# OpenDriveLab/OccNet

Measured on AMD Instinct MI355X. Metric: nuScenes samples/sec (6-cam 900x1600 -> 200x200x16 voxels), higher is better.
Workload: dtype f32 hot path (GEMM operands bf16x3-split, SCA value rows q16 block floating point) + bf16 backbone; 1 GPU; bevformer_base_occ forward: 6x(3x928x1600) images -> ResNet-50+FPN -> 4 BEVFormer layers (TSA+SCA+FFN) -> lifter + 2xConv3d decoder -> 200x200x16 voxels x (17 logits + 2 flow); history_frames=0, mode=infer, scope=e2e, input=resident-f32, samples_per_gpu=1, global_batch=1, parallelism=dp1, step_graph=False, linear_precision=bf16x3, backbone_dtype=bf16

## Files before the change

### include/occnet_amd.h

```cpp
#ifndef OCCNET_AMD_H_
#define OCCNET_AMD_H_

#include <stdint.h>

#ifdef __cplusplus
extern "C" {
#endif

#define OCC_OK 0
#define OCC_E_INVALID (-1)
#define OCC_E_LAUNCH (-2)
#define OCC_E_UNSUPPORTED (-3)

int occ_abi_version(void);
const char* occ_last_error(void);
int occ_selftest_fdiv_f32(const float* a, const float* d, float* q, int64_t n, void* stream);


int occ_ms_deform_attn_forward_f32(const float* value, const int64_t* spatial_shapes,
                                   const int64_t* level_start_index, const float* sampling_loc,
                                   const float* attn_weight, float* out, int B, int S, int M, int D,
                                   int L, int Lq, int P, int im2col_step, void* stream);

int occ_ms_deform_attn_backward_f32(const float* value, const int64_t* spatial_shapes,
// ... 163 lines not shown
int occ_conv_bn_fold_bwd_f32(const void* grad_w_bf16, int64_t stride_o, int64_t stride_i, int64_t stride_h, int64_t stride_w,
                             const float* weight, const float* gamma, const float* rstd, const float* mean_rstd,
                             const float* grad_bias, float* grad_weight, float* grad_gamma, int Cout, int Cin, int KH, int KW,
                             void* stream);

unsigned occ_ln_dropout_hash(unsigned index, unsigned seed_lo, unsigned seed_hi);
int64_t occ_dropout_add_ln_bwd_partial_floats(int64_t rows, int C);
int occ_dropout_add_ln_fwd_f32(const float* x, const float* residual, const float* gamma, const float* beta, float eps,
                               float p_drop, uint64_t seed, float* z, float* y, float* stats, int64_t rows, int C,
                               void* stream);
int occ_dropout_add_ln_bwd_f32(const float* grad_y, const float* z, const float* stats, const float* gamma, float p_drop,
                               uint64_t seed, float* grad_x, float* grad_residual, float* partial, float* grad_gamma_beta,
                               int64_t rows, int C, void* stream);

int64_t occ_bn3d_relu_train_partial_floats(int64_t rows, int C);
int occ_bn3d_relu_train_stats_f32(const float* y, float* partial, float* mean_rstd, float* running_mean, float* running_var,
                                  float eaf, float eps, int64_t rows, int C, void* stream);
int occ_bn3d_relu_train_fwd_f32(const float* y, const float* mean_rstd, const float* gamma, const float* beta, float* out, int B,
                                int Z, int Y, int X, int C, int64_t out_sb, int64_t out_sy, int64_t out_sx, void* stream);
int occ_bn3d_relu_train_bwd_f32(const float* grad_out, int64_t go_sb, int64_t go_sy, int64_t go_sx, const float* y,
                                const float* mean_rstd, const float* gamma, const float* beta, float* partial,
                                float* grad_gamma_beta, float* grad_y, float* grad_y_pad, int B, int Z, int Y, int X, int C,
                                void* stream);

int occ_value_proj_bf16_f32(int n_segments, const void* const* a, const int64_t* lda, const int64_t* rows,
                            const int64_t* rows_per_group, const int64_t* out_row0,
                            const float* const* group_bias, int bias_groups, const void* weight_packed,
                            float* out, int64_t ldo, int K, int N, int64_t out_group_rows, void* stream);
int occ_value_proj_bf16_f16pairs(int n_segments, const void* const* a, const int64_t* lda, const int64_t* rows,
                            const int64_t* rows_per_group, const int64_t* out_row0,
                            const float* const* group_bias, int bias_groups, const void* weight_packed,
                            void* out, int64_t ldo, int K, int N, int64_t out_group_rows, const float* out_scale,
                            void* stream);
int occ_value_proj_bf16_q16pairs(int n_segments, const void* const* a, const int64_t* lda, const int64_t* rows,
                            const int64_t* rows_per_group, const int64_t* out_row0,
                            const float* const* group_bias, int bias_groups, const void* weight_packed,
                            void* out, int64_t ldo, int K, int N, int64_t out_group_rows, const float* out_scale,
                            void* stream);

int occ_value_range_scale_bf16(int n_segments, const void* const* a, const int64_t* lda, const int64_t* rows, int K,
                               int n_planes, const float* row_l1, const float* bias_max, float* scale_out,
                               uint32_t* work, void* stream);
int occ_value_range_scale_from_amax(const uint32_t* amax8, int n_planes, const float* row_l1, const float* bias_max,
                                    float* scale_out, void* stream);

int occ_value_proj_bf16_planes(int n_segments, const void* const* a, const int64_t* lda, const int64_t* rows,
                               const int64_t* rows_per_group, const int64_t* out_row0,
                               const float* const* group_bias, int bias_groups, const void* weight_packed, void* out,
                               int out_f16, int64_t ldo, int K, int n_planes, int plane_cols, int64_t plane_stride,
                               int64_t out_group_rows, const float* out_scale, void* stream);

int occ_stem_conv7x7_pool_f32_bf16(const float* x, const void* weight_frag, const float* bias, void* out,
                                   int batch, int H, int W, void* stream);
int occ_stem_conv7x7_pool_u8_bf16(const uint8_t* x, const void* weight_frag, const float* bias, void* out,
                                  int batch, int Hs, int Ws, int H, int W, const float* mean,
                                  const float* std, int to_rgb, void* stream);

int occ_bias_relu_maxpool_nhwc_bf16(const void* y, const float* bias, void* out, int batch, int H, int W, int C,
                                    void* stream);

int occ_conv1x1_nhwc_bf16(const void* x, const void* weight, const float* bias, const void* residual,
                          void* out, int batch, int Hin, int Win, int Cin, int Cout, int stride, int relu,
                          int residual_upsample2, void* stream);

int occ_conv1x1_nhwc_bf16_variant(const void* x, const void* weight, const float* bias, const void* residual,
                                  void* out, int batch, int Hin, int Win, int Cin, int Cout, int stride, int relu,
                                  int residual_upsample2, int variant, void* stream);

int64_t occ_conv1x1_wgrad_workspace_bytes(int N, int H, int W, int Cin, int Cout, int stride, int splits);
int occ_conv1x1_wgrad_nhwc_bf16(const void* g, const void* x, void* dw, int dw_bf16, void* workspace, int N, int H, int W,
                                int Cin, int Cout, int stride, int splits, void* stream);

int64_t occ_conv3x3_wgrad_workspace_bytes(int N, int H, int W, int Cin, int Cout, int stride, int splits);
int occ_conv3x3_wgrad_nhwc_bf16(const void* g, const void* x, void* dw, int dw_bf16, void* workspace, int N, int H, int W,
                                int Cin, int Cout, int stride, int splits, void* stream);

int occ_conv3x3_pack_weight_bf16(const float* weight, void* packed, int Cout, int Cin, void* stream);
int occ_conv3x3_nhwc_bf16(const void* x, const void* weight_packed, const float* bias, void* out, int batch,
                          int H, int W, int Cin, int Cout, int stride, int relu, void* stream);
int occ_conv3x3_nhwc_bf16_amax(const void* x, const void* weight_packed, const float* bias, void* out, int batch,
                               int H, int W, int Cin, int Cout, int stride, int relu, uint32_t* amax8, void* stream);
int occ_conv3x3_nhwc_bf16_variant(const void* x, const void* weight_packed, const float* bias, void* out, int batch,
                                  int H, int W, int Cin, int Cout, int stride, int relu, uint32_t* amax8, int variant,
                                  void* stream);

int occ_conv3x3_conv1x1_nhwc_bf16(const void* x, const void* w3x3_packed, const float* b2, const void* w1x1_frag,
                                  const float* b3, const void* residual, void* out, int batch, int H, int W, int Cmid,
                                  int Cout, int stride, int variant, void* stream);
int occ_conv3x3_conv1x1_pick(int batch, int H, int W, int Cmid, int Cout, int stride);

int occ_mfma_pack_b_frag_bf16(const float* weight, void* packed, int N, int K, void* stream);

int occ_bottleneck64_nhwc_bf16(const void* x, const void* w1_frag, const float* b1, const void* w2_frag,
                               const float* b2, const void* w3_frag, const float* b3, void* out, int batch,
                               int H, int W, int Cin, int downsample, void* stream);

int occ_bottleneck64_nhwc_bf16_variant(const void* x, const void* w1_frag, const float* b1, const void* w2_frag,
                                       const float* b2, const void* w3_frag, const float* b3, void* out, int batch,
                                       int H, int W, int Cin, int downsample, int variant, void* stream);
int occ_bottleneck64_tile_of_block(int block, int n_blocks, int tiles_x, int tiles_y, int order);

int64_t occ_ray_metrics_state_words(int free_id);
int64_t occ_ray_metrics_workspace_bytes(int B, int X, int Y, int Z);
int occ_ray_metrics_accumulate(const void* sem_pred, int sem_pred_dtype, const float* flow_pred,
                               const void* sem_gt, int sem_gt_dtype, const float* flow_gt,
                               const float* origins, const int32_t* origin_counts, const float* rays,
// ... 26 lines not shown
```

### occnet_amd/csrc/bottleneck64_v2_nhwc_bf16.hip

```cpp
#include "bottleneck64_phases.h"

namespace occ {

constexpr int kBnOS = 32 * kBnMS;
constexpr int kBnBand = 4;

__host__ __device__ inline int bn64_tile_of_block(int block, int n_blocks, int tiles_x, int tiles_y, int order) {
  if (order == 0) return block;
  const int q = n_blocks >> 3, r = n_blocks & 7, x = block & 7, j = block >> 3;
  const int p = x * q + (x < r ? x : r) + j;
  if (order == 1) return p;
  const int per_img = tiles_x * tiles_y, img = p / per_img, pi = p - img * per_img;
  const int r0 = pi / (kBnBand * tiles_x) * kBnBand;
  const int h = tiles_y - r0 < kBnBand ? tiles_y - r0 : kBnBand;
  const int i = pi - r0 * tiles_x;
  return img * per_img + (r0 + i % h) * tiles_x + i / h;
}

template <int CIN, bool DS>
__global__ __launch_bounds__(256, 2) void bottleneck64_v2_nhwc_bf16_kernel(
    const uint4* __restrict__ x, const uint4* __restrict__ w1p, const float* __restrict__ b1,
    const uint4* __restrict__ w2p, const float* __restrict__ b2, const uint4* __restrict__ w3p,
    const float* __restrict__ b3, unsigned short* __restrict__ out, int H, int W, int tiles_x, int tiles_y, int order) {
  static_assert(CIN % 32 == 0 && (DS ? CIN == 64 : CIN == 256), "identity: 4 waves x 2 chunks; projection: both chunks in LDS");
  constexpr int NCH = CIN / 32, CQ = CIN / 8;
  __shared__ __attribute__((aligned(16))) char lds[kBnStageBytes];
  static_assert(4 * kBnOS <= kBnH1, "the waves' epilogue scratch aliases the c1 halo");
  char* const sH1 = lds + 2 * kBnXA;
  char* const sC2 = sH1 + kBnH1;
  const int tid = threadIdx.x, lane = tid & 63, wave = tid >> 6;
  const int vi = lane & 31, kb = lane >> 5;
  const int tile = bn64_tile_of_block((int)blockIdx.x, (int)gridDim.x, tiles_x, tiles_y, order);
  OCC_BN_TILE_DECODE(tile)

  OCC_BN_STAGING
  const int rot = DS ? 0 : (int)(((unsigned)tile * 5u) % (unsigned)NCH);

  OCC_BN_WAVE_TILES
  float4 bA[4], bB[4];
  OCC_BN_ZERO_ACC(acc1, 3)
  uint2 idn[2][4][4];
  const int wave_u = __builtin_amdgcn_readfirstlane(wave);
  const int cbase = (((vi >> 4) + 1) * kBnHW + (vi & 15) + 1) * kBnXS + 8 * kb;
#define OCC_B2_CAPTURE(T, SX)                                                                     \
  _Pragma("unroll") for (int rt = 0; rt < 4; ++rt)                                                \
    _Pragma("unroll") for (int q = 0; q < 4; ++q)                                                 \
      idn[T][rt][q] = *reinterpret_cast<const uint2*>((SX) + cbase + rt * (2 * kBnHW * kBnXS) + 16 * q);
  constexpr int WD = 3;
  uint4 wa[WD][2];
  OCC_BN_ISSUE_W1(0, OCC_BN_CH(0))
  OCC_BN_ISSUE_X(0, OCC_BN_CH(0))
  OCC_BN_ISSUE_W1(1, OCC_BN_CH(NCH > 1 ? 1 : 0))
  OCC_BN_ISSUE_X(1, OCC_BN_CH(NCH > 1 ? 1 : 0))
  if (NCH > 2) {
    OCC_BN_ISSUE_W1(2, OCC_BN_CH(NCH > 2 ? 2 : 0))
    OCC_BN_ISSUE_X(2, OCC_BN_CH(NCH > 2 ? 2 : 0))
    OCC_BN_ISSUE_X(3, OCC_BN_CH(NCH > 3 ? 3 : 0))
  }
#define OCC_B2_STEP_A(S, CI)                                                                      \
  {                                                                                               \
    char* sX = lds + ((CI) & 1) * kBnXA;                                                          \
    OCC_BN_STAGE_STORE(S, sX)                                                                     \
    OCC_BN_W1_FRAGS((CI) % WD)                                                                    \
    __syncthreads();                                                                              \
    if ((CI) + WD < NCH) OCC_BN_ISSUE_W1((CI) % WD, OCC_BN_CH((CI) + WD < NCH ? (CI) + WD : NCH - 1)) \
    if ((CI) + 4 < NCH) OCC_BN_ISSUE_X(S, OCC_BN_CH((CI) + 4 < NCH ? (CI) + 4 : NCH - 1))         \
    if ((CI) == NCH - 2) { OCC_BN_ISSUE_BIASES }                                                  \
    OCC_BN_STEP_MFMA(sX)                                                                          \
    if (!DS) {                                                                                    \
// ... 95 lines not shown
```

### occnet_amd/csrc/common.h

```cpp
#pragma once
#include <hip/hip_runtime.h>
#include <stdint.h>
#include <stdio.h>
#include <stdlib.h>
#include "../../include/occnet_amd.h"

namespace occ {

void set_error(const char* fmt, ...);
#define OCC_CHECK_ARG(cond, ...)              \
  do {                                        \
    if (!(cond)) {                            \
      ::occ::set_error(__VA_ARGS__);          \
      return OCC_E_INVALID;                   \
    }                                         \
  } while (0)
#define OCC_CHECK_LAUNCH(what)                                                  \
  do {                                                                          \
    hipError_t e__ = hipGetLastError();                                         \
    if (e__ != hipSuccess) {                                                    \
      ::occ::set_error("%s: launch failed: %s", what, hipGetErrorString(e__));  \
      return OCC_E_LAUNCH;                                                      \
    }                                                                           \
  } while (0)
// ... 44 lines not shown
  return t.c[0] + t.c[1] + t.c[2] + t.c[3];
}

__device__ __forceinline__ unsigned pack_bf16x2_rne(float lo, float hi) {
  typedef float occ_f32x2 __attribute__((ext_vector_type(2)));
  typedef __bf16 occ_bf16x2 __attribute__((ext_vector_type(2)));
  const occ_f32x2 v = {lo, hi};
  return __builtin_bit_cast(unsigned, __builtin_convertvector(v, occ_bf16x2));
}
__device__ __forceinline__ unsigned short bf16_rne(float f) {
  return (unsigned short)(pack_bf16x2_rne(f, 0.f) & 0xffffu);
}

__device__ __forceinline__ float bf16_to_f32(unsigned short h) { return __uint_as_float((unsigned)h << 16); }
__device__ __forceinline__ float bf16_lo_to_f32(unsigned v) { return __uint_as_float(v << 16); }
__device__ __forceinline__ float bf16_hi_to_f32(unsigned v) { return __uint_as_float(v & 0xffff0000u); }

__device__ __forceinline__ void bf16_split(float x, unsigned short& hi, unsigned short& lo) {
  hi = bf16_rne(x);
  lo = bf16_rne(x - bf16_to_f32(hi));
}
__device__ __forceinline__ void bf16_split2(float x0, float x1, unsigned& hi, unsigned& lo) {
  hi = pack_bf16x2_rne(x0, x1);
  lo = pack_bf16x2_rne(x0 - bf16_lo_to_f32(hi), x1 - bf16_hi_to_f32(hi));
}

typedef float f32x16 __attribute__((ext_vector_type(16)));
typedef __bf16 bf16x8 __attribute__((ext_vector_type(8)));
typedef unsigned short u16x2 __attribute__((ext_vector_type(2)));
typedef unsigned occ_u32x4 __attribute__((ext_vector_type(4)));
typedef __attribute__((address_space(3))) void* lds_ptr_t;

__device__ __forceinline__ float wave_sum(float v) {
#pragma unroll
  for (int d = 32; d >= 1; d >>= 1) v += __shfl_xor(v, d);
  return v;
}

__device__ __forceinline__ unsigned absmax_pk2(unsigned m, unsigned x) {
  const u16x2 a = __builtin_bit_cast(u16x2, m), b = __builtin_bit_cast(u16x2, x & 0x7fff7fffu);
  return __builtin_bit_cast(unsigned, __builtin_elementwise_max(a, b));
}

__device__ __forceinline__ float softplus(float x) {
  const float e = __builtin_amdgcn_exp2f(fabsf(x) * -1.44269504088896341f);
  return fmaxf(x, 0.f) + __builtin_amdgcn_logf(1.f + e) * 0.693147180559945309f;
}

inline bool env_default_on(const char* name) {
  const char* e = getenv(name);
  return !(e && e[0] == '0');
}

__device__ __forceinline__ float fdiv(float a, float d) {
  float r = __builtin_amdgcn_rcpf(d);
  r = fmaf(fmaf(-d, r, 1.f), r, r);
  const float q = a * r;
  const float c = fmaf(fmaf(-q, d, a), r, q);
  return fabsf(q) < __builtin_huge_valf() ? c : q;
}

__device__ __forceinline__ void wave_lds_sync() {
  __builtin_amdgcn_fence(__ATOMIC_RELEASE, "wavefront");
  __builtin_amdgcn_wave_barrier();
  __builtin_amdgcn_fence(__ATOMIC_ACQUIRE, "wavefront");
}

template <int UNROLL>
__device__ __forceinline__ float4 gather_samples(const float* __restrict__ vb,
                                                 const SampleParam* sp, int ns, float4 acc) {
  int s = 0;
  for (; s + UNROLL <= ns; s += UNROLL) {
    float4 w[UNROLL];
    int4 o[UNROLL];
#pragma unroll
    for (int u = 0; u < UNROLL; ++u) {
      w[u] = *reinterpret_cast<const float4*>(sp[s + u].w);
      o[u] = *reinterpret_cast<const int4*>(sp[s + u].o);
    }
    float4 v[UNROLL][4];
#pragma unroll
    for (int u = 0; u < UNROLL; ++u) {
      v[u][0] = *reinterpret_cast<const float4*>(vb + o[u].x);
      v[u][1] = *reinterpret_cast<const float4*>(vb + o[u].y);
      v[u][2] = *reinterpret_cast<const float4*>(vb + o[u].z);
      v[u][3] = *reinterpret_cast<const float4*>(vb + o[u].w);
    }
#pragma unroll
    for (int u = 0; u < UNROLL; ++u) {
      const float ww[4] = {w[u].x, w[u].y, w[u].z, w[u].w};
#pragma unroll
      for (int k = 0; k < 4; ++k) {
        acc.x = fmaf(ww[k], v[u][k].x, acc.x);
        acc.y = fmaf(ww[k], v[u][k].y, acc.y);
        acc.z = fmaf(ww[k], v[u][k].z, acc.z);
        acc.w = fmaf(ww[k], v[u][k].w, acc.w);
      }
    }
  }
  for (; s < ns; ++s) {
    const float4 w = *reinterpret_cast<const float4*>(sp[s].w);
    const int4 o = *reinterpret_cast<const int4*>(sp[s].o);
    const float4 v0 = *reinterpret_cast<const float4*>(vb + o.x);
    const float4 v1 = *reinterpret_cast<const float4*>(vb + o.y);
    const float4 v2 = *reinterpret_cast<const float4*>(vb + o.z);
    const float4 v3 = *reinterpret_cast<const float4*>(vb + o.w);
// ... 166 lines not shown
```

### occnet_amd/csrc/stem_conv7x7_pool.hip

```cpp
#include "common.h"

namespace occ {

constexpr int kStP = 8;
constexpr int kStC = 2 * kStP + 1;
constexpr int kStI = 2 * kStC + 5;
constexpr int kStIW = 40;
constexpr int kStIn = kStI * kStIW * 8;
constexpr int kStNC = kStC * kStC;
constexpr int kStMS = 144;
constexpr int kStConv = 320 * kStMS;

struct StemNorm { float mean[3], stdinv[3]; int Hs, Ws, to_rgb; };

template <bool U8>
__global__ __launch_bounds__(256, 2) void stem_conv7x7_pool_kernel(
    const void* __restrict__ x_, const uint4* __restrict__ wfrag, const float* __restrict__ bias,
    uint4* __restrict__ out, int H, int W, int Hc, int Wc, int Hp, int Wp, int tiles_x, int tiles_y,
    StemNorm nrm) {
  __shared__ __attribute__((aligned(16))) char lds[kStIn + kStConv];
  char* const sIn = lds;
  char* const sCv = lds + kStIn;
  const int tid = threadIdx.x, lane = tid & 63, wave = tid >> 6;
  const int vi = lane & 31, kb = lane >> 5;
  int bid = blockIdx.x;
  const int tx_i = bid % tiles_x; bid /= tiles_x;
  const int ty_i = bid % tiles_y;
  const int img = bid / tiles_y;
  const int py0 = ty_i * kStP, px0 = tx_i * kStP;
  const int cy0 = 2 * py0 - 1, cx0 = 2 * px0 - 1;
  const int iy0 = 2 * cy0 - 3, ix0 = 2 * cx0 - 3;

  const int nt = wave & 1, mt0 = 5 * (wave >> 1);
  uint4 wf[14];
#pragma unroll
  for (int s = 0; s < 14; ++s) wf[s] = wfrag[((long)s * 2 + nt) * 64 + lane];
  float4 bv[4];
#pragma unroll
  for (int g = 0; g < 4; ++g) bv[g] = *reinterpret_cast<const float4*>(bias + nt * 32 + 8 * g + 4 * kb);

  {
    const long plane = (long)H * W;
    const float* xi = reinterpret_cast<const float*>(x_) + (long)img * 3 * plane;
    const unsigned char* xu = reinterpret_cast<const unsigned char*>(x_) + (long)img * nrm.Hs * nrm.Ws * 3;
    constexpr int ITEMS = 4 * kStI * kStIW;
    constexpr int NJ = (ITEMS + 255) / 256;
    float v[NJ];
#pragma unroll
    for (int j = 0; j < NJ; ++j) {
      const int idx = min(tid + 256 * j, ITEMS - 1);
      const int c = idx / (kStI * kStIW), r = idx % (kStI * kStIW);
      const int ly = r / kStIW, lx = r % kStIW;
      const int cc = c < 3 ? c : 0, cy = min(max(iy0 + ly, 0), H - 1), cx = min(max(ix0 + lx, 0), W - 1);
      if (U8) {
        const int sy = min(cy, nrm.Hs - 1), sx = min(cx, nrm.Ws - 1), sc = nrm.to_rgb ? 2 - cc : cc;
        const float raw = (float)xu[((long)sy * nrm.Ws + sx) * 3 + sc];
        const float mu = cc == 0 ? nrm.mean[0] : (cc == 1 ? nrm.mean[1] : nrm.mean[2]);
        const float si = cc == 0 ? nrm.stdinv[0] : (cc == 1 ? nrm.stdinv[1] : nrm.stdinv[2]);
        v[j] = (cy < nrm.Hs && cx < nrm.Ws) ? (raw - mu) * si : 0.f;
      } else {
        v[j] = xi[cc * plane + (long)cy * W + cx];
      }
    }
#pragma unroll
    for (int j = 0; j < NJ; ++j) {
      const int idx = tid + 256 * j;
      if (idx < ITEMS) {
        const int c = idx / (kStI * kStIW), r = idx % (kStI * kStIW);
        const int ly = r / kStIW, lx = r % kStIW;
        const int iy = iy0 + ly, ix = ix0 + lx;
        const bool in = c < 3 && lx < kStI && iy >= 0 && iy < H && ix >= 0 && ix < W;
        *reinterpret_cast<unsigned short*>(sIn + (ly * kStIW + lx) * 8 + c * 2) = in ? bf16_rne(v[j]) : (unsigned short)0;
      }
    }
  }
  __syncthreads();

  int abase[5];
  bool cvalid[5];
#pragma unroll
  for (int j = 0; j < 5; ++j) {
    const int q = (mt0 + j) * 32 + vi;
    const int qc = q < kStNC ? q : kStNC - 1;
    const int cyl = qc / kStC, cxl = qc - cyl * kStC;
    abase[j] = ((2 * cyl) * kStIW + 2 * cxl) * 8 + kb * 16;
    const int cy = cy0 + cyl, cx = cx0 + cxl;
    cvalid[j] = q < kStNC && cy >= 0 && cy < Hc && cx >= 0 && cx < Wc;
  }
  f32x16 acc[5];
#pragma unroll
  for (int j = 0; j < 5; ++j)
#pragma unroll
    for (int r = 0; r < 16; ++r) acc[j][r] = 0.f;
#pragma unroll
  for (int s = 0; s < 14; ++s) {
    const int koff = (s >> 1) * (kStIW * 8) + (s & 1) * 32;
    const bf16x8 w = __builtin_bit_cast(bf16x8, wf[s]);
#pragma unroll
    for (int j = 0; j < 5; ++j) {
      const bf16x8 a = *reinterpret_cast<const bf16x8*>(sIn + abase[j] + koff);
      acc[j] = __builtin_amdgcn_mfma_f32_32x32x16_bf16(w, a, acc[j], 0, 0, 0);
    }
  }
#pragma unroll
  for (int j = 0; j < 5; ++j) {
    const int q = (mt0 + j) * 32 + vi;
    if (q < kStNC) {
      const float m = cvalid[j] ? 1.f : 0.f;
      char* dst = sCv + q * kStMS + (nt * 32 + 4 * kb) * 2;
#pragma unroll
      for (int g = 0; g < 4; ++g) {
        const float v0 = fmaxf(acc[j][4 * g + 0] + bv[g].x, 0.f) * m, v1 = fmaxf(acc[j][4 * g + 1] + bv[g].y, 0.f) * m;
        const float v2 = fmaxf(acc[j][4 * g + 2] + bv[g].z, 0.f) * m, v3 = fmaxf(acc[j][4 * g + 3] + bv[g].w, 0.f) * m;
        *reinterpret_cast<uint2*>(dst + 16 * g) = make_uint2(pack_bf16x2_rne(v0, v1), pack_bf16x2_rne(v2, v3));
      }
    }
  }
  __syncthreads();

#pragma unroll
  for (int j = 0; j < 2; ++j) {
    const int item = tid + 256 * j;
    const int cg = item & 7, p = item >> 3;
    const int pyl = p >> 3, pxl = p & 7;
    const int py = py0 + pyl, px = px0 + pxl;
    if (py < Hp && px < Wp) {
      float m[8];
#pragma unroll
      for (int k = 0; k < 8; ++k) m[k] = 0.f;
#pragma unroll
      for (int dy = 0; dy < 3; ++dy)
#pragma unroll
        for (int dx = 0; dx < 3; ++dx) {
          const uint4 v = *reinterpret_cast<const uint4*>(sCv + ((2 * pyl + dy) * kStC + 2 * pxl + dx) * kStMS + cg * 16);
          const unsigned vv[4] = {v.x, v.y, v.z, v.w};
#pragma unroll
          for (int k = 0; k < 4; ++k) {
            m[2 * k] = fmaxf(m[2 * k], __uint_as_float(vv[k] << 16));
            m[2 * k + 1] = fmaxf(m[2 * k + 1], __uint_as_float(vv[k] & 0xffff0000u));
          }
        }
      out[(((long)img * Hp + py) * Wp + px) * 8 + cg] =
          make_uint4(pack_bf16x2_rne(m[0], m[1]), pack_bf16x2_rne(m[2], m[3]), pack_bf16x2_rne(m[4], m[5]),
                     pack_bf16x2_rne(m[6], m[7]));
    }
  }
}

}

extern "C" int occ_stem_conv7x7_pool_f32_bf16(const float* x, const void* weight_frag, const float* bias,
                                              void* out, int batch, int H, int W, void* stream) {
  using namespace occ;
  OCC_CHECK_ARG(x && weight_frag && bias && out, "stem_conv7x7_pool: null pointer argument");
  OCC_CHECK_ARG(batch > 0 && H > 0 && W > 0, "stem_conv7x7_pool: bad dimension");
  const int Hc = (H - 1) / 2 + 1, Wc = (W - 1) / 2 + 1;
  const int Hp = (Hc - 1) / 2 + 1, Wp = (Wc - 1) / 2 + 1;
  const int tiles_x = (Wp + kStP - 1) / kStP, tiles_y = (Hp + kStP - 1) / kStP;
  hipLaunchKernelGGL(stem_conv7x7_pool_kernel<false>, dim3((unsigned)((long)batch * tiles_x * tiles_y)), dim3(256), 0,
                     reinterpret_cast<hipStream_t>(stream), x, reinterpret_cast<const uint4*>(weight_frag), bias,
                     reinterpret_cast<uint4*>(out), H, W, Hc, Wc, Hp, Wp, tiles_x, tiles_y, StemNorm{});
  OCC_CHECK_LAUNCH("stem_conv7x7_pool");
  return OCC_OK;
}

extern "C" int occ_stem_conv7x7_pool_u8_bf16(const uint8_t* x, const void* weight_frag, const float* bias,
                                             void* out, int batch, int Hs, int Ws, int H, int W,
                                             const float* mean, const float* std, int to_rgb, void* stream) {
  using namespace occ;
  OCC_CHECK_ARG(x && weight_frag && bias && out && mean && std, "stem_conv7x7_pool_u8: null pointer argument");
  OCC_CHECK_ARG(batch > 0 && Hs > 0 && Ws > 0 && H >= Hs && W >= Ws, "stem_conv7x7_pool_u8: bad dimension");
  OCC_CHECK_ARG(std[0] != 0.f && std[1] != 0.f && std[2] != 0.f, "stem_conv7x7_pool_u8: zero std");
  const int Hc = (H - 1) / 2 + 1, Wc = (W - 1) / 2 + 1;
  const int Hp = (Hc - 1) / 2 + 1, Wp = (Wc - 1) / 2 + 1;
  const int tiles_x = (Wp + kStP - 1) / kStP, tiles_y = (Hp + kStP - 1) / kStP;
  StemNorm nrm;
  for (int c = 0; c < 3; ++c) { nrm.mean[c] = mean[c]; nrm.stdinv[c] = (float)(1.0 / (double)std[c]); }
  nrm.Hs = Hs; nrm.Ws = Ws; nrm.to_rgb = to_rgb ? 1 : 0;
  hipLaunchKernelGGL(stem_conv7x7_pool_kernel<true>, dim3((unsigned)((long)batch * tiles_x * tiles_y)), dim3(256), 0,
                     reinterpret_cast<hipStream_t>(stream), x, reinterpret_cast<const uint4*>(weight_frag), bias,
                     reinterpret_cast<uint4*>(out), H, W, Hc, Wc, Hp, Wp, tiles_x, tiles_y, nrm);
  OCC_CHECK_LAUNCH("stem_conv7x7_pool_u8");
  return OCC_OK;
}
```

### occnet_amd/ext.py

```python
import ctypes
import os

import torch

from . import _lib, cache_epoch
from ._lib import OccAmdError, OccAmdUnsupported, f32, i32, i64, ptr, stream_ptr


_TIMING = None
_TIMING_ONLY = None


def kernel_timing(enable=True):
    global _TIMING, _TIMING_ONLY
    _TIMING = {} if enable else None
    _TIMING_ONLY = None
    return _TIMING


def kernel_timing_only(names):
    global _TIMING_ONLY
    _TIMING_ONLY = None if names is None else set(names)


# ... 1844 lines not shown
    nfl = int(lib.occ_bias_act_bwd_partial_floats(i64(rows), i32(C)))
    if nfl <= 0:
        raise OccAmdUnsupported(f"bias_act_bwd_nhwc: no kernel for C={C}")
    partial = torch.empty(nfl, dtype=torch.float32, device=grad_y.device)
    bias_grad = torch.empty(C, dtype=torch.float32, device=grad_y.device)
    g = torch.empty_like(grad_y) if relu else grad_y
    with torch.cuda.device(grad_y.device):
        rc = _lib.lib().occ_bias_act_bwd_nhwc_bf16(ptr(grad_y), ptr(y) if relu else ptr(None), ptr(g) if relu else ptr(None),
                                                   ptr(partial), ptr(bias_grad), i64(rows), i32(C), i32(1 if relu else 0),
                                                   stream_ptr(grad_y.device))
    _lib.check(rc, "bias_act_bwd_nhwc")
    return g, bias_grad


def conv_bn_fold_fwd(weight, gamma, beta, rstd, mean_rstd):
    for n, t in (("weight", weight), ("gamma", gamma), ("beta", beta), ("rstd", rstd), ("mean_rstd", mean_rstd)):
        _need_cuda_f32(n, t)
    O, I, KH, KW = weight.shape
    wf = torch.empty_like(weight, memory_format=torch.contiguous_format)
    w16 = torch.empty((O, I, KH, KW), dtype=torch.bfloat16, device=weight.device, memory_format=torch.channels_last)
    b = torch.empty(O, dtype=torch.float32, device=weight.device)
    with torch.cuda.device(weight.device):
        rc = _lib.lib().occ_conv_bn_fold_fwd_f32(ptr(weight), ptr(gamma), ptr(beta), ptr(rstd), ptr(mean_rstd), ptr(wf), ptr(w16),
                                                 ptr(b), i32(O), i32(I), i32(KH), i32(KW), stream_ptr(weight.device))
    _lib.check(rc, "conv_bn_fold_fwd")
    return wf, w16, b


def conv_bn_fold_bwd(grad_w16, weight, gamma, rstd, mean_rstd, grad_bias):
    if not (grad_w16.is_cuda and grad_w16.dtype == torch.bfloat16 and grad_w16.shape == weight.shape):
        raise OccAmdUnsupported("conv_bn_fold_bwd: grad_w16 must be a bfloat16 device tensor of the weight's shape")
    for n, t in (("weight", weight), ("gamma", gamma), ("rstd", rstd), ("mean_rstd", mean_rstd), ("grad_bias", grad_bias)):
        _need_cuda_f32(n, t)
    O, I, KH, KW = weight.shape
    dW = torch.empty_like(weight, memory_format=torch.contiguous_format)
    dgamma = torch.empty(O, dtype=torch.float32, device=weight.device)
    so, si, sh, sw = grad_w16.stride()
    with torch.cuda.device(weight.device):
        rc = _lib.lib().occ_conv_bn_fold_bwd_f32(ptr(grad_w16), i64(so), i64(si), i64(sh), i64(sw), ptr(weight), ptr(gamma),
                                                 ptr(rstd), ptr(mean_rstd), ptr(grad_bias), ptr(dW), ptr(dgamma), i32(O), i32(I),
                                                 i32(KH), i32(KW), stream_ptr(weight.device))
    _lib.check(rc, "conv_bn_fold_bwd")
    return dW, dgamma


def stem_pack_weight(weight):
    if tuple(weight.shape) != (64, 3, 7, 7):
        raise OccAmdUnsupported("stem_pack_weight: expected a (64, 3, 7, 7) weight")
    w2 = torch.zeros(64, 7, 8, 4, dtype=torch.float32, device=weight.device)
    w2[:, :, :7, :3] = weight.float().permute(0, 2, 3, 1)
    return mfma_pack_b_frag(w2.reshape(64, 224))


def stem_conv7x7_pool(x, weight_frag, bias):
    _need_cuda_f32("x", x)
    _need_cuda_f32("bias", bias)
    if x.dim() != 4 or x.shape[1] != 3 or not x.is_contiguous():
        raise OccAmdUnsupported("stem_conv7x7_pool: x must be a contiguous (N, 3, H, W) fp32 tensor")
    if weight_frag.numel() != 64 * 224 or bias.numel() != 64:
        raise OccAmdError("stem_conv7x7_pool: inconsistent shapes")
    N, _, H, W = x.shape
    Hc, Wc = (H - 1) // 2 + 1, (W - 1) // 2 + 1
    Hp, Wp = (Hc - 1) // 2 + 1, (Wc - 1) // 2 + 1
    out = torch.empty((N, 64, Hp, Wp), dtype=torch.bfloat16, device=x.device, memory_format=torch.channels_last)
    with torch.cuda.device(x.device), _timed('bb_stem7x7_pool'):
        rc = _lib.lib().occ_stem_conv7x7_pool_f32_bf16(ptr(x), ptr(weight_frag), ptr(bias), ptr(out), i32(N),
                                                       i32(H), i32(W), stream_ptr(x.device))
    _note_flops('bb_stem7x7_pool', 2.0 * N * Hc * Wc * 64 * 147)
    _lib.check(rc, "stem_conv7x7_pool")
    return out


def stem_conv7x7_pool_u8(x_u8, weight_frag, bias, mean, std, to_rgb=False, size_divisor=32):
    if not (x_u8.is_cuda and x_u8.dtype == torch.uint8 and x_u8.dim() == 4 and x_u8.shape[-1] == 3
            and x_u8.is_contiguous()):
        raise OccAmdUnsupported("stem_conv7x7_pool_u8: x must be a contiguous (N, H, W, 3) uint8 device tensor")
    _need_cuda_f32("bias", bias)
    if weight_frag.numel() != 64 * 224 or bias.numel() != 64:
        raise OccAmdError("stem_conv7x7_pool_u8: inconsistent shapes")
    N, Hs, Ws, _ = x_u8.shape
    d = int(size_divisor)
    H, W = (Hs + d - 1) // d * d, (Ws + d - 1) // d * d
    Hc, Wc = (H - 1) // 2 + 1, (W - 1) // 2 + 1
    Hp, Wp = (Hc - 1) // 2 + 1, (Wc - 1) // 2 + 1
    out = torch.empty((N, 64, Hp, Wp), dtype=torch.bfloat16, device=x_u8.device, memory_format=torch.channels_last)
    mean_c = (f32 * 3)(*[float(v) for v in mean])
    std_c = (f32 * 3)(*[float(v) for v in std])
    with torch.cuda.device(x_u8.device):
        rc = _lib.lib().occ_stem_conv7x7_pool_u8_bf16(ptr(x_u8), ptr(weight_frag), ptr(bias), ptr(out), i32(N),
                                                      i32(Hs), i32(Ws), i32(H), i32(W), mean_c, std_c,
                                                      i32(1 if to_rgb else 0), stream_ptr(x_u8.device))
    _lib.check(rc, "stem_conv7x7_pool_u8")
    return out, (H, W)


def bias_relu_maxpool_nhwc(y, bias):
    _need_cl_bf16("bias_relu_maxpool_nhwc", "y", y)
    _need_cuda_f32("bias", bias)
    N, C, H, W = y.shape
    if bias.numel() != C:
        raise OccAmdError("bias_relu_maxpool_nhwc: bias must have C entries")
    out = torch.empty((N, C, (H - 1) // 2 + 1, (W - 1) // 2 + 1), dtype=torch.bfloat16, device=y.device,
                      memory_format=torch.channels_last)
    with torch.cuda.device(y.device):
        rc = _lib.lib().occ_bias_relu_maxpool_nhwc_bf16(ptr(y), ptr(bias), ptr(out), i32(N), i32(H), i32(W),
                                                        i32(C), stream_ptr(y.device))
    _lib.check(rc, "bias_relu_maxpool_nhwc")
    return out


def conv1x1_pack_weight(weight2d):
    cout, cin = weight2d.shape
    if cin % 32 or cout % 32:
        raise OccAmdUnsupported("conv1x1_pack_weight: Cin and Cout must be multiples of 32")
    return mfma_pack_b_frag(weight2d.float().contiguous())


def conv1x1_nhwc(x, weight_frag, bias, residual=None, relu=False, stride=1, residual_upsample2=False, variant=None,
                 _timing='bb_conv1x1'):
    _need_cl_bf16("conv1x1_nhwc", "x", x)
# ... 244 lines not shown
```

Baseline: 188.0 samples/s.

## Add second stem conv7x7+pool kernel with float4 loads, LDS pool and XCD tile order

Adds a second fused stem conv7x7+maxpool kernel and routes the f32 input to it by default when W is a multiple of 4 and x is 16-byte aligned. It loads the input as float4 per channel plane, writes the conv output to LDS (aliased over the input tile) and does the 3x3 max pool there with packed bf16 max. It also uses an XCD-aware banded tile order (default order 1) shared with the bottleneck kernel, and raises occupancy to 3 blocks per SM. The goal is less global-load overhead and better L2 locality in the stem, at the cost of a new code path plus env switches and probe tools.

```diff
diff --git a/include/occnet_amd.h b/include/occnet_amd.h
--- a/include/occnet_amd.h
+++ b/include/occnet_amd.h
@@ -239,6 +239,10 @@
 
 int occ_stem_conv7x7_pool_f32_bf16(const float* x, const void* weight_frag, const float* bias, void* out,
                                    int batch, int H, int W, void* stream);
+int occ_stem_conv7x7_pool_f32_bf16_variant(const float* x, const void* weight_frag, const float* bias, void* out,
+                                           int batch, int H, int W, int variant, void* stream);
+int occ_stem_route(const float* x, int W, int variant);
+int occ_stem_tile_of_block(int block, int n_blocks, int tiles_x, int tiles_y, int order);
 int occ_stem_conv7x7_pool_u8_bf16(const uint8_t* x, const void* weight_frag, const float* bias, void* out,
                                   int batch, int Hs, int Ws, int H, int W, const float* mean,
                                   const float* std, int to_rgb, void* stream);
diff --git a/occnet_amd/csrc/bottleneck64_v2_nhwc_bf16.hip b/occnet_amd/csrc/bottleneck64_v2_nhwc_bf16.hip
--- a/occnet_amd/csrc/bottleneck64_v2_nhwc_bf16.hip
+++ b/occnet_amd/csrc/bottleneck64_v2_nhwc_bf16.hip
@@ -6,15 +6,7 @@
 constexpr int kBnBand = 4;
 
 __host__ __device__ inline int bn64_tile_of_block(int block, int n_blocks, int tiles_x, int tiles_y, int order) {
-  if (order == 0) return block;
-  const int q = n_blocks >> 3, r = n_blocks & 7, x = block & 7, j = block >> 3;
-  const int p = x * q + (x < r ? x : r) + j;
-  if (order == 1) return p;
-  const int per_img = tiles_x * tiles_y, img = p / per_img, pi = p - img * per_img;
-  const int r0 = pi / (kBnBand * tiles_x) * kBnBand;
-  const int h = tiles_y - r0 < kBnBand ? tiles_y - r0 : kBnBand;
-  const int i = pi - r0 * tiles_x;
-  return img * per_img + (r0 + i % h) * tiles_x + i / h;
+  return xcd_tile_of_block(block, n_blocks, tiles_x, tiles_y, order, kBnBand);
 }
 
 template <int CIN, bool DS>
diff --git a/occnet_amd/csrc/common.h b/occnet_amd/csrc/common.h
--- a/occnet_amd/csrc/common.h
+++ b/occnet_amd/csrc/common.h
@@ -120,6 +120,18 @@
   return !(e && e[0] == '0');
 }
 
+__host__ __device__ inline int xcd_tile_of_block(int block, int n_blocks, int tiles_x, int tiles_y, int order, int band) {
+  if (order == 0) return block;
+  const int q = n_blocks >> 3, r = n_blocks & 7, x = block & 7, j = block >> 3;
+  const int p = x * q + (x < r ? x : r) + j;
+  if (order == 1) return p;
+  const int per_img = tiles_x * tiles_y, img = p / per_img, pi = p - img * per_img;
+  const int r0 = pi / (band * tiles_x) * band;
+  const int h = tiles_y - r0 < band ? tiles_y - r0 : band;
+  const int i = pi - r0 * tiles_x;
+  return img * per_img + (r0 + i % h) * tiles_x + i / h;
+}
+
 __device__ __forceinline__ float fdiv(float a, float d) {
   float r = __builtin_amdgcn_rcpf(d);
   r = fmaf(fmaf(-d, r, 1.f), r, r);
diff --git a/occnet_amd/csrc/stem_conv7x7_pool.hip b/occnet_amd/csrc/stem_conv7x7_pool.hip
--- a/occnet_amd/csrc/stem_conv7x7_pool.hip
+++ b/occnet_amd/csrc/stem_conv7x7_pool.hip
@@ -12,6 +12,34 @@
 constexpr int kStConv = 320 * kStMS;
 
 struct StemNorm { float mean[3], stdinv[3]; int Hs, Ws, to_rgb; };
+
+__device__ __forceinline__ void stem_conv_tiles(const char* sIn, const uint4 (&wf)[14], int mt0, int vi, int kb, int cy0,
+                                                int cx0, int Hc, int Wc, bool (&cvalid)[5], f32x16 (&acc)[5]) {
+  int abase[5];
+#pragma unroll
+  for (int j = 0; j < 5; ++j) {
+    const int q = (mt0 + j) * 32 + vi;
+    const int qc = q < kStNC ? q : kStNC - 1;
+    const int cyl = qc / kStC, cxl = qc - cyl * kStC;
+    abase[j] = ((2 * cyl) * kStIW + 2 * cxl) * 8 + kb * 16;
+    const int cy = cy0 + cyl, cx = cx0 + cxl;
+    cvalid[j] = q < kStNC && cy >= 0 && cy < Hc && cx >= 0 && cx < Wc;
+  }
+#pragma unroll
+  for (int j = 0; j < 5; ++j)
+#pragma unroll
+    for (int r = 0; r < 16; ++r) acc[j][r] = 0.f;
+#pragma unroll
+  for (int s = 0; s < 14; ++s) {
+    const int koff = (s >> 1) * (kStIW * 8) + (s & 1) * 32;
+    const bf16x8 w = __builtin_bit_cast(bf16x8, wf[s]);
+#pragma unroll
+    for (int j = 0; j < 5; ++j) {
+      const bf16x8 a = *reinterpret_cast<const bf16x8*>(sIn + abase[j] + koff);
+      acc[j] = __builtin_amdgcn_mfma_f32_32x32x16_bf16(w, a, acc[j], 0, 0, 0);
+    }
+  }
+}
 
 template <bool U8>
 __global__ __launch_bounds__(256, 2) void stem_conv7x7_pool_kernel(
@@ -76,32 +104,9 @@
   }
   __syncthreads();
 
-  int abase[5];
   bool cvalid[5];
-#pragma unroll
-  for (int j = 0; j < 5; ++j) {
-    const int q = (mt0 + j) * 32 + vi;
-    const int qc = q < kStNC ? q : kStNC - 1;
-    const int cyl = qc / kStC, cxl = qc - cyl * kStC;
-    abase[j] = ((2 * cyl) * kStIW + 2 * cxl) * 8 + kb * 16;
-    const int cy = cy0 + cyl, cx = cx0 + cxl;
-    cvalid[j] = q < kStNC && cy >= 0 && cy < Hc && cx >= 0 && cx < Wc;
-  }
   f32x16 acc[5];
-#pragma unroll
-  for (int j = 0; j < 5; ++j)
-#pragma unroll
-    for (int r = 0; r < 16; ++r) acc[j][r] = 0.f;
-#pragma unroll
-  for (int s = 0; s < 14; ++s) {
-    const int koff = (s >> 1) * (kStIW * 8) + (s & 1) * 32;
-    const bf16x8 w = __builtin_bit_cast(bf16x8, wf[s]);
-#pragma unroll
-    for (int j = 0; j < 5; ++j) {
-      const bf16x8 a = *reinterpret_cast<const bf16x8*>(sIn + abase[j] + koff);
-      acc[j] = __builtin_amdgcn_mfma_f32_32x32x16_bf16(w, a, acc[j], 0, 0, 0);
-    }
-  }
+  stem_conv_tiles(sIn, wf, mt0, vi, kb, cy0, cx0, Hc, Wc, cvalid, acc);
 #pragma unroll
   for (int j = 0; j < 5; ++j) {
     const int q = (mt0 + j) * 32 + vi;
@@ -147,21 +152,178 @@
   }
 }
 
-}
-
-extern "C" int occ_stem_conv7x7_pool_f32_bf16(const float* x, const void* weight_frag, const float* bias,
-                                              void* out, int batch, int H, int W, void* stream) {
-  using namespace occ;
+constexpr int kStItemsX = 11;
+constexpr int kStItems = kStI * kStItemsX;
+constexpr int kStBand = 4;
+typedef unsigned short u16x8 __attribute__((ext_vector_type(8)));
+
+__global__ __launch_bounds__(256, 3) void stem_conv7x7_pool_v2_kernel(
+    const float* __restrict__ x, const uint4* __restrict__ wfrag, const float* __restrict__ bias,
+    uint4* __restrict__ out, int H, int W, int Hc, int Wc, int Hp, int Wp, int tiles_x, int tiles_y, int order) {
+  static_assert(kStIn <= kStConv, "the conv tile covers the input tile");
+  __shared__ __attribute__((aligned(16))) char lds[kStConv];
+  char* const sIn = lds;
+  char* const sCv = lds;
+  const int tid = threadIdx.x, lane = tid & 63, wave = tid >> 6;
+  const int vi = lane & 31, kb = lane >> 5;
+  int bid = xcd_tile_of_block((int)blockIdx.x, (int)gridDim.x, tiles_x, tiles_y, order, kStBand);
+  const int tx_i = bid % tiles_x; bid /= tiles_x;
+  const int ty_i = bid % tiles_y;
+  const int img = bid / tiles_y;
+  const int py0 = ty_i * kStP, px0 = tx_i * kStP;
+  const int cy0 = 2 * py0 - 1, cx0 = 2 * px0 - 1;
+  const int iy0 = 2 * cy0 - 3, ix0 = 2 * cx0 - 3;
+
+  const int nt = wave & 1, mt0 = 5 * (wave >> 1);
+  uint4 wf[14];
+#pragma unroll
+  for (int s = 0; s < 14; ++s) wf[s] = wfrag[((long)s * 2 + nt) * 64 + lane];
+
+  {
+    const long plane = (long)H * W;
+    const float* xi = x + (long)img * 3 * plane;
+    constexpr int NJ = (kStItems + 255) / 256;
+    float4 v[NJ][3];
+#pragma unroll
+    for (int j = 0; j < NJ; ++j) {
+      const int i = tid + 256 * j;
+      const int ly = i / kStItemsX, k = i - ly * kStItemsX;
+      const int iy = iy0 + ly, gx = ix0 - 3 + 4 * k;
+      const bool in = i < kStItems && iy >= 0 && iy < H && gx >= 0 && gx < W;
+      const float* p = xi + (long)iy * W + gx;
+#pragma unroll
+      for (int c = 0; c < 3; ++c)
+        v[j][c] = in ? *reinterpret_cast<const float4*>(p + c * plane) : make_float4(0.f, 0.f, 0.f, 0.f);
+    }
+#pragma unroll
+    for (int j = 0; j < NJ; ++j) {
+      const int i = tid + 256 * j;
+      const int ly = i / kStItemsX, k = i - ly * kStItemsX;
+      if (i < kStItems) {
+        const float4 a = v[j][0], b = v[j][1], c = v[j][2];
+        const uint2 p0 = make_uint2(pack_bf16x2_rne(a.x, b.x), pack_bf16x2_rne(c.x, 0.f));
+        const uint2 p1 = make_uint2(pack_bf16x2_rne(a.y, b.y), pack_bf16x2_rne(c.y, 0.f));
+        uint2 p2 = make_uint2(pack_bf16x2_rne(a.z, b.z), pack_bf16x2_rne(c.z, 0.f));
+        const uint2 p3 = make_uint2(pack_bf16x2_rne(a.w, b.w), pack_bf16x2_rne(c.w, 0.f));
+        if (k == kStItemsX - 1) p2 = make_uint2(0u, 0u);
+        char* d = sIn + (ly * kStIW + 4 * k - 3) * 8;
+        if (k > 0) {
+          *reinterpret_cast<uint2*>(d) = p0;
+          *reinterpret_cast<uint4*>(d + 8) = make_uint4(p1.x, p1.y, p2.x, p2.y);
+        }
+        if (k < kStItemsX - 1) *reinterpret_cast<uint2*>(d + 24) = p3;
+      }
+    }
+  }
+  __syncthreads();
+
+  bool cvalid[5];
+  f32x16 acc[5];
+  stem_conv_tiles(sIn, wf, mt0, vi, kb, cy0, cx0, Hc, Wc, cvalid, acc);
+  float4 bv[4];
+#pragma unroll
+  for (int g = 0; g < 4; ++g) bv[g] = *reinterpret_cast<const float4*>(bias + nt * 32 + 8 * g + 4 * kb);
+  __syncthreads();
+#pragma unroll
+  for (int j = 0; j < 5; ++j) {
+    const int q = (mt0 + j) * 32 + vi;
+    if (q < kStNC) {
+      char* dst = sCv + q * kStMS + (nt * 32 + 4 * kb) * 2;
+#pragma unroll
+      for (int g = 0; g < 4; ++g) {
+        const float v0 = fmaxf(acc[j][4 * g + 0] + bv[g].x, 0.f), v1 = fmaxf(acc[j][4 * g + 1] + bv[g].y, 0.f);
+        const float v2 = fmaxf(acc[j][4 * g + 2] + bv[g].z, 0.f), v3 = fmaxf(acc[j][4 * g + 3] + bv[g].w, 0.f);
+        *reinterpret_cast<uint2*>(dst + 16 * g) =
+            cvalid[j] ? make_uint2(pack_bf16x2_rne(v0, v1), pack_bf16x2_rne(v2, v3)) : make_uint2(0u, 0u);
+      }
+    }
+  }
+  __syncthreads();
+
+#pragma unroll
+  for (int j = 0; j < 2; ++j) {
+    const int item = tid + 256 * j;
+    const int cg = item & 7, p = item >> 3;
+    const int pyl = p >> 3, pxl = p & 7;
+    const int py = py0 + pyl, px = px0 + pxl;
+    if (py < Hp && px < Wp) {
+      const char* src = sCv + ((2 * pyl) * kStC + 2 * pxl) * kStMS + cg * 16;
+      u16x8 m = *reinterpret_cast<const u16x8*>(src);
+#pragma unroll
+      for (int t = 1; t < 9; ++t)
+        m = __builtin_elementwise_max(m, *reinterpret_cast<const u16x8*>(src + ((t / 3) * kStC + t % 3) * kStMS));
+      out[(((long)img * Hp + py) * Wp + px) * 8 + cg] = __builtin_bit_cast(uint4, m);
+    }
+  }
+}
+
+constexpr int kStVariantDefault = 4;
+
+static int stem_route(const float* x, int W, int variant) {
+  if (variant < 0 || variant > 5) {
+    set_error("stem_conv7x7_pool: no variant %d (0 = default, 1 = first kernel, 2 = second kernel, 3, 4, 5 = second kernel "
+              "with tile order 0, 1, 2)", variant);
+    return OCC_E_INVALID;
+  }
+  static const bool v2_on = env_default_on("OCC_STEM_V2");
+  static const int v2_default = [] {
+    const char* e = getenv("OCC_STEM_VARIANT");
+    return e && e[0] >= '3' && e[0] <= '5' && !e[1] ? e[0] - '0' : kStVariantDefault;
+  }();
+  const bool fits = W % 4 == 0 && reinterpret_cast<uintptr_t>(x) % 16 == 0;
+  if (variant == 0) variant = v2_on && fits ? 2 : 1;
+  if (variant == 2) variant = v2_default;
+  if (variant != 1 && !fits) {
+    set_error("stem_conv7x7_pool: the second kernel needs W %% 4 == 0 and a 16-byte-aligned x (W = %d)", W);
+    return OCC_E_UNSUPPORTED;
+  }
+  return variant;
+}
+
+static int stem_launch(const float* x, const void* weight_frag, const float* bias, void* out, int batch, int H, int W,
+                       int variant, void* stream) {
   OCC_CHECK_ARG(x && weight_frag && bias && out, "stem_conv7x7_pool: null pointer argument");
   OCC_CHECK_ARG(batch > 0 && H > 0 && W > 0, "stem_conv7x7_pool: bad dimension");
+  const int route = stem_route(x, W, variant);
+  if (route < 0) return route;
   const int Hc = (H - 1) / 2 + 1, Wc = (W - 1) / 2 + 1;
   const int Hp = (Hc - 1) / 2 + 1, Wp = (Wc - 1) / 2 + 1;
   const int tiles_x = (Wp + kStP - 1) / kStP, tiles_y = (Hp + kStP - 1) / kStP;
-  hipLaunchKernelGGL(stem_conv7x7_pool_kernel<false>, dim3((unsigned)((long)batch * tiles_x * tiles_y)), dim3(256), 0,
-                     reinterpret_cast<hipStream_t>(stream), x, reinterpret_cast<const uint4*>(weight_frag), bias,
-                     reinterpret_cast<uint4*>(out), H, W, Hc, Wc, Hp, Wp, tiles_x, tiles_y, StemNorm{});
+  const dim3 grid((unsigned)((long)batch * tiles_x * tiles_y));
+  hipStream_t st = reinterpret_cast<hipStream_t>(stream);
+  const uint4* wf = reinterpret_cast<const uint4*>(weight_frag);
+  uint4* o = reinterpret_cast<uint4*>(out);
+  if (route == 1)
+    hipLaunchKernelGGL(stem_conv7x7_pool_kernel<false>, grid, dim3(256), 0, st, x, wf, bias, o, H, W, Hc, Wc, Hp, Wp,
+                       tiles_x, tiles_y, StemNorm{});
+  else
+    hipLaunchKernelGGL(stem_conv7x7_pool_v2_kernel, grid, dim3(256), 0, st, x, wf, bias, o, H, W, Hc, Wc, Hp, Wp,
+                       tiles_x, tiles_y, route - 3);
   OCC_CHECK_LAUNCH("stem_conv7x7_pool");
   return OCC_OK;
+}
+
+}
+
+extern "C" int occ_stem_conv7x7_pool_f32_bf16(const float* x, const void* weight_frag, const float* bias,
+                                              void* out, int batch, int H, int W, void* stream) {
+  return occ::stem_launch(x, weight_frag, bias, out, batch, H, W, 0, stream);
+}
+
+extern "C" int occ_stem_conv7x7_pool_f32_bf16_variant(const float* x, const void* weight_frag, const float* bias,
+                                                      void* out, int batch, int H, int W, int variant, void* stream) {
+  return occ::stem_launch(x, weight_frag, bias, out, batch, H, W, variant, stream);
+}
+
+extern "C" int occ_stem_route(const float* x, int W, int variant) { return occ::stem_route(x, W, variant); }
+
+extern "C" int occ_stem_tile_of_block(int block, int n_blocks, int tiles_x, int tiles_y, int order) {
+  using namespace occ;
+  OCC_CHECK_ARG(tiles_x > 0 && tiles_y > 0 && n_blocks > 0 && n_blocks % (tiles_x * tiles_y) == 0,
+                "stem_tile_of_block: n_blocks must be a positive multiple of tiles_x * tiles_y");
+  OCC_CHECK_ARG(block >= 0 && block < n_blocks, "stem_tile_of_block: block outside 0 .. n_blocks - 1");
+  OCC_CHECK_ARG(order >= 0 && order <= 2, "stem_tile_of_block: order must be 0, 1 or 2");
+  return xcd_tile_of_block(block, n_blocks, tiles_x, tiles_y, order, kStBand);
 }
 
 extern "C" int occ_stem_conv7x7_pool_u8_bf16(const uint8_t* x, const void* weight_frag, const float* bias,
diff --git a/occnet_amd/ext.py b/occnet_amd/ext.py
--- a/occnet_amd/ext.py
+++ b/occnet_amd/ext.py
@@ -1920,7 +1920,7 @@
     return mfma_pack_b_frag(w2.reshape(64, 224))
 
 
-def stem_conv7x7_pool(x, weight_frag, bias):
+def stem_conv7x7_pool(x, weight_frag, bias, variant=0):
     _need_cuda_f32("x", x)
     _need_cuda_f32("bias", bias)
     if x.dim() != 4 or x.shape[1] != 3 or not x.is_contiguous():
@@ -1932,8 +1932,8 @@
     Hp, Wp = (Hc - 1) // 2 + 1, (Wc - 1) // 2 + 1
     out = torch.empty((N, 64, Hp, Wp), dtype=torch.bfloat16, device=x.device, memory_format=torch.channels_last)
     with torch.cuda.device(x.device), _timed('bb_stem7x7_pool'):
-        rc = _lib.lib().occ_stem_conv7x7_pool_f32_bf16(ptr(x), ptr(weight_frag), ptr(bias), ptr(out), i32(N),
-                                                       i32(H), i32(W), stream_ptr(x.device))
+        rc = _lib.lib().occ_stem_conv7x7_pool_f32_bf16_variant(ptr(x), ptr(weight_frag), ptr(bias), ptr(out), i32(N),
+                                                               i32(H), i32(W), i32(int(variant)), stream_ptr(x.device))
     _note_flops('bb_stem7x7_pool', 2.0 * N * Hc * Wc * 64 * 147)
     _lib.check(rc, "stem_conv7x7_pool")
     return out
diff --git a/tools_dev/stem_pmc.py b/tools_dev/stem_pmc.py
--- /dev/null
+++ b/tools_dev/stem_pmc.py
@@ -0,0 +1,73 @@
+#!/usr/bin/env python
+import argparse
+import collections
+import csv
+import glob
+import os
+import subprocess
+import sys
+import tempfile
+
+SETS = ["FETCH_SIZE", "WRITE_SIZE", "TCC_HIT_sum TCC_MISS_sum", "SQ_WAVE_CYCLES SQ_WAIT_INST_ANY SQ_BUSY_CYCLES",
+        "SQ_INSTS_VALU SQ_ACTIVE_INST_VALU SQ_INSTS_LDS", "SQ_VALU_MFMA_BUSY_CYCLES TA_TA_BUSY_sum",
+        "SQ_LDS_BANK_CONFLICT SQ_LDS_IDX_ACTIVE"]
+ROOT = os.path.dirname(os.path.dirname(os.path.abspath(__file__)))
+
+
+def main():
+    ap = argparse.ArgumentParser()
+    ap.add_argument('--variants', default='1,3,4,5')
+    ap.add_argument('--out', default=None, help='also write the table to this file')
+    a = ap.parse_args()
+    variants = [int(v) for v in a.variants.split(',')]
+    iters = 2
+    order = [1] + variants + [v for v in variants for _ in range(3 + iters)]
+    acc = collections.defaultdict(lambda: [0, 0.0])
+    notes = []
+    for cset in SETS:
+        d = tempfile.mkdtemp(prefix='stempmc_')
+        cmd = ['rocprofv3', '--pmc'] + cset.split() + ['--kernel-trace', '--output-format', 'csv',
+               '--kernel-include-regex', 'stem_conv7x7', '-d', d, '-o', 'p', '--', sys.executable,
+               os.path.join(ROOT, 'tools_dev', 'stem_probe.py'), '--variants', a.variants, '--iters', str(iters),
+               '--rounds', '1']
+        try:
+            res = subprocess.run(cmd, capture_output=True, text=True, timeout=240, cwd=d)
+        except subprocess.TimeoutExpired:
+            raise SystemExit(f"rocprofv3 ran into its time limit on counter set {cset!r}: stopping")
+        if res.returncode < 0 or res.returncode in (124, 134, 137, 139):
+            sys.stderr.write(res.stdout[-2000:] + res.stderr[-2000:])
+            raise SystemExit(f"rocprofv3 ended with {res.returncode} on counter set {cset!r}: stopping")
+        paths = glob.glob(os.path.join(d, '**', '*counter_collection.csv'), recursive=True)
+        if res.returncode != 0 or not paths:
+            notes.append(f"# counter set {cset!r}: not collected (exit {res.returncode}): "
+                         + (res.stderr.strip().splitlines() or ['no output'])[-1][:160])
+            continue
+        rows = [r for p in paths for r in csv.DictReader(open(p))]
+        ids = sorted({int(r['Dispatch_Id']) for r in rows if 'stem_conv7x7' in r['Kernel_Name']})
+        if len(ids) != len(order):
+            raise SystemExit(f"{len(ids)} stem launches, expected {len(order)}")
+        which = dict(zip(ids, order))
+        for r in rows:
+            if 'stem_conv7x7' in r['Kernel_Name']:
+                v = which[int(r['Dispatch_Id'])]
+                assert ('_v2_' in r['Kernel_Name']) == (v != 1), (r['Kernel_Name'], v)
+                k = acc[(v, r['Counter_Name'])]
+                k[0] += 1
+                k[1] += float(r['Counter_Value'])
+    lines = ["# rocprofv3 --pmc (one counter set per run, kernel trace only) over tools_dev/stem_probe.py, 6 x 3 x 928 x 1600;",
+             "# mean per launch.  variant 1 = first kernel, 3 / 4 / 5 = second kernel with tile order 0 / 1 / 2.",
+             "# FETCH_SIZE / WRITE_SIZE in KB as rocprofv3 reports them"] + notes
+    names = sorted({c for (_, c) in acc})
+    lines.append(f"  {'counter':28s}" + ''.join(f"{'variant ' + str(v):>16s}" for v in variants))
+    for c in names:
+        lines.append(f"  {c:28s}" + ''.join(f"{acc[(v, c)][1] / max(acc[(v, c)][0], 1):16.5g}" for v in variants))
+    text = '\n'.join(lines) + '\n'
+    if a.out:
+        os.makedirs(os.path.dirname(os.path.abspath(a.out)), exist_ok=True)
+        with open(a.out, 'w') as f:
+            f.write(text)
+    print(text)
+
+
+if __name__ == '__main__':
+    main()
diff --git a/tools_dev/stem_probe.py b/tools_dev/stem_probe.py
--- /dev/null
+++ b/tools_dev/stem_probe.py
@@ -0,0 +1,39 @@
+import argparse
+import os
+import sys
+sys.path.insert(0, os.path.join(os.path.dirname(os.path.abspath(__file__)), ".."))
+import torch
+from occnet_amd import ext
+
+
+def run(variants, iters, rounds):
+    g = torch.Generator().manual_seed(0)
+    N, H, W = 6, 928, 1600
+    x = (torch.randn(N, 3, H, W, generator=g) * 50.0).cuda()
+    frag = ext.stem_pack_weight((torch.randn(64, 3, 7, 7, generator=g) / 12.0).cuda())
+    b = torch.randn(64, generator=g).cuda()
+    ref = ext.stem_conv7x7_pool(x, frag, b, variant=1)
+    mb = (x.numel() * 4 + ref.numel() * 2) / 1e6
+    for v in variants:
+        same = torch.equal(ext.stem_conv7x7_pool(x, frag, b, variant=v), ref)
+        print(f"stem variant {v}: bits equal to variant 1: {same}")
+    for r in range(rounds):
+        for v in variants:
+            for _ in range(3):
+                ext.stem_conv7x7_pool(x, frag, b, variant=v)
+            a, e = torch.cuda.Event(enable_timing=True), torch.cuda.Event(enable_timing=True)
+            torch.cuda.synchronize(); a.record()
+            for _ in range(iters):
+                ext.stem_conv7x7_pool(x, frag, b, variant=v)
+            e.record(); torch.cuda.synchronize()
+            us = a.elapsed_time(e) * 1e3 / iters
+            print(f"stem variant {v} round {r}: {us:.1f} us  ({mb:.0f} MB min traffic -> {mb / us:.2f} TB/s)", flush=True)
+
+
+if __name__ == '__main__':
+    ap = argparse.ArgumentParser()
+    ap.add_argument('--variants', default='1,2')
+    ap.add_argument('--iters', type=int, default=50)
+    ap.add_argument('--rounds', type=int, default=5)
+    a = ap.parse_args()
+    run([int(v) for v in a.variants.split(',')], a.iters, a.rounds)
```

After: 189.9 samples/s (median of 6 runs). No clear change (+1.0%).
